# nv-tlabs/GEN3C

Measured on NVIDIA H100. Metric: denoise-steps/sec, 7B DiT, 121-frame 720p latent, higher is better.
Workload: dtype bf16

## Files before the change

### gen3c_b200/_lib.py

```python
from __future__ import annotations

import ctypes as C
import os
from pathlib import Path

_HERE = Path(__file__).resolve().parent
LIB_PATH = _HERE / "lib" / "libgen3c_b200.so"


class G3CError(RuntimeError):
    pass


class DitConfig(C.Structure):
    _fields_ = [
        ("model_channels", C.c_int),
        ("num_blocks", C.c_int),
        ("num_heads", C.c_int),
        ("ffn_dim", C.c_int),
        ("context_dim", C.c_int),
        ("adaln_lora_dim", C.c_int),
        ("in_channels", C.c_int),
        ("out_channels", C.c_int),
        ("concat_padding_mask", C.c_int),
# ... 23 lines not shown
        ("sigma_data", C.c_float),
        ("sigma_aug", C.c_float),
        ("guidance", C.c_float),
        ("xt_next", C.c_void_p),
        ("cond_mask_uncond", C.c_void_p),
        ("net_output", C.c_void_p),
    ]


_P = C.c_void_p
_I = C.c_int
_F = C.c_float

SIGNATURES = {
    "g3c_last_error": (C.c_char_p, []),
    "g3c_version": (_I, []),
    "g3c_device_info": (_I, [C.POINTER(_I), C.POINTER(_I), C.POINTER(_I)]),
    "g3c_render_create": (_I, [_I, _I, _I, C.POINTER(_P)]),
    "g3c_render_destroy": (_I, [_P]),
    "g3c_render_set_deterministic": (_I, [_P, _I]),
    "g3c_forward_warp": (_I, [_P, _P, _P, _P, _P, _P, _I, _I, _I, _P, _P, _P, _P, _P]),
    "g3c_render_cache": (_I, [_P, _P, _P, _P, _P, _P, _I, _I, _I, _I, _I, _P, _P, _P, _P]),
    "g3c_bilinear_splatting": (_I, [_P, _P, _P, _P, _P, _I, _I, _I, _P, _P, _P]),
    "g3c_splat_indices": (_I, [_P, _I, _I, _I, _P, _P]),
    "g3c_unproject_points": (_I, [_P, _P, _P, _P, _I, _I, _I, _I, _P, _P]),
    "g3c_reliable_depth_mask": (_I, [_P, _I, _I, _I, _I, _F, _F, _P, _P]),
    "g3c_align_depth_nonrigid": (_I, [_P, _P, _P, _P, _P, _I, _I, _I, _F, _F, _P, _P]),
    "g3c_foreground_occlusion": (_I, [_P, _P, _P, _P, _I, _I, _I, _I, _P, _P, _P, _P]),
    "g3c_render_cache_occlusion": (_I, [_P, _P, _P, _P, _I, _I, _I, _I, _P, _P, _P, _I, _I, _P]),
    "g3c_gemm_bf16": (_I, [_P, _P, _P, _I, _I, _I, _I, _I, _I, _I, _P, _I, _P]),
    "g3c_gemm_norm_rope_bf16": (_I, [_P, _P, _P, _I, _I, _I, _I, _I, _I, _P, _P, _F, _P]),
    "g3c_quantize_rows_fp8": (_I, [_P, _I, _I, _I, _P, _I, _P, _P]),
    "g3c_gemm_fp8": (_I, [_P, _P, _P, _P, _P, _I, _I, _I, _I, _I, _I, _I, _P, _I, _P]),
    "g3c_gemm_norm_rope_fp8": (_I, [_P, _P, _P, _P, _P, _I, _I, _I, _I, _I, _I, _P, _P, _F, _P]),
    "g3c_ln_modulate_fp8": (_I, [_P, _P, _P, _P, _P, _P, _I, _I, _F, _P]),
    "g3c_attn_fwd": (_I, [_P, _P, _P, _P, _I, _I, _I, _I, _I, _I, _I, _F, _P]),
    "g3c_attn_fwd_sbhd": (_I, [_P, _P, _P, _P, _I, _I, _I, _I, _I, _I, _I, _I, _F, _P]),
    "g3c_attn_set_trace": (_I, [_P]),
    "g3c_ln_modulate": (_I, [_P, _P, _P, _P, _P, _I, _I, _F, _P]),
    "g3c_rmsnorm_rope": (_I, [_P, _I, _I, _I, _P, _P, _F, _P]),
    "g3c_dit_create": (_I, [C.POINTER(DitConfig), C.POINTER(_P)]),
    "g3c_dit_destroy": (_I, [_P]),
    "g3c_dit_load": (_I, [_P, C.c_char_p, _P, C.POINTER(C.c_int64), _I, _I]),
    "g3c_nccl_unique_id": (_I, [_P]),
    "g3c_dit_enable_cp": (_I, [_P, _P, _I, _I]),
    "g3c_dit_cp_export": (_I, [_P, _P]),
    "g3c_dit_cp_import": (_I, [_P, _P, _I]),
    "g3c_dit_cp_mode": (_I, [_P]),
    "g3c_dit_disable_cp": (_I, [_P]),
    "g3c_dit_set_linear_fp8": (_I, [_P, _I]),
    "g3c_dit_enable_cfg_parallel": (_I, [_P, _I]),
    "g3c_dit_cfg_export": (_I, [_P, _P]),
    "g3c_dit_cfg_import": (_I, [_P, _P]),
    "g3c_dit_set_shape": (_I, [_P, _I, _I, _I, _I, _F]),
    "g3c_dit_forward": (_I, [_P, _P, _P, _P, _P, _F, _P, _P, _P]),
    "g3c_denoise_step": (_I, [_P, C.POINTER(StepArgs), _P]),
    "g3c_dit_profile": (_I, [_P, _I]),
    "g3c_dit_profile_read": (_I, [_P, C.POINTER(_F), C.POINTER(_I), _I]),
    "g3c_dit_profile_wait_ms": (_I, [_P, C.POINTER(_F)]),
    "g3c_dit_workspace_bytes": (C.c_int64, [_P]),
    "g3c_dit_last_launch_count": (_I, [_P]),
    "g3c_dit_read_tables": (_I, [_P, _I, _P, _P, _P]),
    "g3c_dit_read_modulation": (_I, [_P, _F, _P, _P, _P]),
    "g3c_dit_read_step": (_I, [_P, _P, _P, _P, _P, _P]),
    "g3c_attn_fwd_gated": (_I, [_P, _P, _P, _P, _I, _I, _I, _I, _I, _I, _I, _F, _P, C.c_uint32, _I, _P, _P]),
}

# ... 41 lines not shown
```

### gen3c_b200/csrc/common.cuh

```cuda
#pragma once
#include <cuda.h>
#include <cuda_bf16.h>
#include <cuda_runtime.h>
#include <stdint.h>
#include <stdio.h>

#include "../../include/gen3c_b200.h"
#include "wgmma_ops.cuh"

namespace g3c {

void set_error(const char* fmt, ...);
int cuda_fail(cudaError_t e, const char* what, const char* file, int line);
#define G3C_CUDA(x)                                                         \
  do {                                                                      \
    cudaError_t _e = (x);                                                   \
    if (_e != cudaSuccess) return ::g3c::cuda_fail(_e, #x, __FILE__, __LINE__); \
  } while (0)
#define G3C_REQUIRE(cond, ...)        \
  do {                                \
    if (!(cond)) {                    \
      ::g3c::set_error(__VA_ARGS__);  \
      return G3C_EINVAL;       \
    }                                 \
// ... 11 lines not shown
__device__ __forceinline__ uint32_t smem_u32(const void* p) {
  return static_cast<uint32_t>(__cvta_generic_to_shared(p));
}
__device__ __forceinline__ uint32_t lane_id() { return threadIdx.x & 31; }
__device__ __forceinline__ uint32_t warp_id() { return __shfl_sync(0xffffffffu, threadIdx.x >> 5, 0); }

__device__ __forceinline__ bool elect_one() {
  uint32_t pred = 0;
  asm volatile(
      "{\n\t.reg .pred P;\n\t"
      "elect.sync _|P, 0xffffffff;\n\t"
      "selp.b32 %0, 1, 0, P;\n\t}\n"
      : "=r"(pred));
  return pred != 0;
}

__device__ __forceinline__ void mbar_init(uint64_t* bar, uint32_t count) {
  asm volatile("mbarrier.init.shared::cta.b64 [%0], %1;\n" ::"r"(smem_u32(bar)), "r"(count));
}
__device__ __forceinline__ void fence_barrier_init() {
  asm volatile("fence.mbarrier_init.release.cluster;\n" ::: "memory");
}
__device__ __forceinline__ void fence_proxy_async() {
  asm volatile("fence.proxy.async.shared::cta;\n" ::: "memory");
}
__device__ __forceinline__ void mbar_expect_tx(uint64_t* bar, uint32_t bytes) {
  asm volatile("mbarrier.arrive.expect_tx.shared::cta.b64 _, [%0], %1;\n" ::"r"(smem_u32(bar)),
               "r"(bytes)
               : "memory");
}
__device__ __forceinline__ void mbar_arrive(uint64_t* bar) {
  asm volatile("mbarrier.arrive.shared::cta.b64 _, [%0];\n" ::"r"(smem_u32(bar)) : "memory");
}
#ifndef G3C_MBAR_SUSPEND_NS
#define G3C_MBAR_SUSPEND_NS 0
#endif
__device__ __forceinline__ bool mbar_try_wait(uint64_t* bar, uint32_t parity) {
  uint32_t ok;
#if G3C_MBAR_SUSPEND_NS > 0
  asm volatile(
      "{\n\t.reg .pred P;\n\t"
      "mbarrier.try_wait.parity.shared::cta.b64 P, [%1], %2, %3;\n\t"
      "selp.b32 %0, 1, 0, P;\n\t}\n"
      : "=r"(ok)
      : "r"(smem_u32(bar)), "r"(parity), "r"((uint32_t)G3C_MBAR_SUSPEND_NS)
      : "memory");
#else
  asm volatile(
      "{\n\t.reg .pred P;\n\t"
      "mbarrier.try_wait.parity.shared::cta.b64 P, [%1], %2;\n\t"
      "selp.b32 %0, 1, 0, P;\n\t}\n"
      : "=r"(ok)
      : "r"(smem_u32(bar)), "r"(parity)
      : "memory");
#endif
  return ok != 0;
}
__device__ __forceinline__ bool mbar_test(uint64_t* bar, uint32_t parity) {
  uint32_t ok;
  asm volatile(
      "{\n\t.reg .pred P;\n\t"
      "mbarrier.test_wait.parity.shared::cta.b64 P, [%1], %2;\n\t"
      "selp.b32 %0, 1, 0, P;\n\t}\n"
      : "=r"(ok)
      : "r"(smem_u32(bar)), "r"(parity)
      : "memory");
  return ok != 0;
}
#ifndef G3C_MBAR_TIMEOUT_NS
#define G3C_MBAR_TIMEOUT_NS 4000000000ull
#endif
__device__ __forceinline__ uint64_t global_timer_ns() {
  uint64_t t;
  asm volatile("mov.u64 %0, %%globaltimer;\n" : "=l"(t));
  return t;
}
#ifdef G3C_MBAR_DEBUG
#define G3C_MBAR_TIMEOUT_ACTION(bar, parity)                                                                 \
  do {                                                                                                       \
    printf("g3c: mbarrier timeout block(%d,%d) thread %d bar@%u parity %u\n", blockIdx.x, blockIdx.y,        \
           threadIdx.x, bar, parity);                                                                        \
    __trap();                                                                                                \
  } while (0)
#else
#define G3C_MBAR_TIMEOUT_ACTION(bar, parity) asm volatile("trap;\n")
#endif
__device__ __forceinline__ void mbar_wait(uint64_t* bar, uint32_t parity) {
  if (mbar_try_wait(bar, parity)) return;
  uint32_t spins = 0;
  uint64_t t0 = 0;
  while (!mbar_try_wait(bar, parity)) {
    if ((++spins & 0xFFFu) == 0) {
      uint64_t now = global_timer_ns();
      if (t0 == 0) t0 = now;
      else if (now - t0 > G3C_MBAR_TIMEOUT_NS) G3C_MBAR_TIMEOUT_ACTION(smem_u32(bar), parity);
    }
  }
}

__device__ __forceinline__ void mbar_wait_ns(uint64_t* bar, uint32_t parity, unsigned long long timeout_ns) {
  if (mbar_try_wait(bar, parity)) return;
  uint32_t spins = 0;
  uint64_t t0 = 0;
  while (!mbar_try_wait(bar, parity)) {
    if ((++spins & 0xFFFu) == 0) {
      uint64_t now = global_timer_ns();
      if (t0 == 0) t0 = now;
      else if (now - t0 > timeout_ns) G3C_MBAR_TIMEOUT_ACTION(smem_u32(bar), parity);
    }
  }
}

__device__ __forceinline__ void mbar_wait_ns_or_exit(uint64_t* bar, uint32_t parity, unsigned long long timeout_ns) {
  if (mbar_try_wait(bar, parity)) return;
  uint32_t spins = 0;
  uint64_t t0 = 0;
  while (!mbar_try_wait(bar, parity)) {
    if ((++spins & 0xFFFu) == 0) {
      uint64_t now = global_timer_ns();
      if (t0 == 0) t0 = now;
      else if (now - t0 > timeout_ns) asm volatile("exit;\n");
    }
  }
}

__device__ __forceinline__ void tma_prefetch_desc(const CUtensorMap* m) {
  asm volatile("prefetch.tensormap [%0];\n" ::"l"(reinterpret_cast<uint64_t>(m)) : "memory");
}
__device__ __forceinline__ void tma_load_2d(void* smem_dst, const CUtensorMap* m, uint64_t* bar,
                                            int c0, int c1) {
  asm volatile(
      "cp.async.bulk.tensor.2d.shared::cluster.global.mbarrier::complete_tx::bytes"
      " [%0], [%1, {%3, %4}], [%2];\n" ::"r"(smem_u32(smem_dst)),
      "l"(reinterpret_cast<uint64_t>(m)), "r"(smem_u32(bar)), "r"(c0), "r"(c1)
      : "memory");
}
__device__ __forceinline__ void tma_load_3d(void* smem_dst, const CUtensorMap* m, uint64_t* bar,
                                            int c0, int c1, int c2) {
  asm volatile(
      "cp.async.bulk.tensor.3d.shared::cluster.global.mbarrier::complete_tx::bytes"
      " [%0], [%1, {%3, %4, %5}], [%2];\n" ::"r"(smem_u32(smem_dst)),
      "l"(reinterpret_cast<uint64_t>(m)), "r"(smem_u32(bar)), "r"(c0), "r"(c1), "r"(c2)
      : "memory");
}

__device__ __forceinline__ void tma_store_2d(const CUtensorMap* m, const void* smem_src, int c0, int c1) {
  asm volatile("cp.async.bulk.tensor.2d.global.shared::cta.bulk_group [%0, {%2, %3}], [%1];\n" ::"l"(
                   reinterpret_cast<uint64_t>(m)),
               "r"(smem_u32(smem_src)), "r"(c0), "r"(c1)
               : "memory");
}
__device__ __forceinline__ void tma_reduce_add_2d(const CUtensorMap* m, const void* smem_src, int c0, int c1) {
  asm volatile("cp.reduce.async.bulk.tensor.2d.global.shared::cta.add.bulk_group [%0, {%2, %3}], [%1];\n" ::"l"(
                   reinterpret_cast<uint64_t>(m)),
               "r"(smem_u32(smem_src)), "r"(c0), "r"(c1)
               : "memory");
}
__device__ __forceinline__ void tma_store_commit() { asm volatile("cp.async.bulk.commit_group;\n" ::: "memory"); }
template <int N>
__device__ __forceinline__ void tma_store_wait_read() {
  asm volatile("cp.async.bulk.wait_group.read %0;\n" ::"n"(N) : "memory");
}
template <int N>
__device__ __forceinline__ void tma_store_wait_all() {
  asm volatile("cp.async.bulk.wait_group %0;\n" ::"n"(N) : "memory");
}

__device__ __forceinline__ void wgmma_fence() { asm volatile("wgmma.fence.sync.aligned;\n" ::: "memory"); }
__device__ __forceinline__ void wgmma_commit() { asm volatile("wgmma.commit_group.sync.aligned;\n" ::: "memory"); }
// ... 62 lines not shown
```

### gen3c_b200/csrc/gemm_wgmma.cu

```cuda
#include <cstdlib>
#include <cstring>

#include "kernels.h"

namespace g3c {

constexpr int BM = 128;
constexpr int BK = 64;
constexpr int WG_K = 16;
template <bool kFp8>
constexpr int kBlockK = kFp8 ? 2 * BK : BK;
constexpr int GEMM_THREADS = 384;

struct GemmParams {
  int M, N, K;
  int ldd;
  void* D;
  const float* gate;
  int num_m_blk, num_n_blk, num_k_blk;
  int super_n;
  const float* nr_gamma;
  const float* nr_cs;
  float nr_eps;
  const float* scale_a;
  const float* scale_b;
};

constexpr int EPI_NORM_ROPE_BF16 = 4;

template <int BN>
struct GemmSmem {
  static constexpr int kABytes = BM * BK * 2;
  static constexpr int kBBytes = BN * BK * 2;
  static constexpr int kStageBytes = kABytes + kBBytes;
  static constexpr int kStages = (192 * 1024) / kStageBytes;
  static constexpr int kBarBytes = 256;
  static constexpr int kTotal = kStages * kStageBytes + kBarBytes + 1024;
};

__device__ __forceinline__ float gelu_erf(float x) {
  return 0.5f * x * (1.0f + erff(x * 0.70710678118654752440f));
}

__device__ __forceinline__ void tile_coords(const GemmParams& p, int tile, int& m_blk, int& n_blk) {
  int per_super = p.num_m_blk * p.super_n;
  int sc = tile / per_super;
  int rem = tile - sc * per_super;
  int n0 = sc * p.super_n;
  int width = p.num_n_blk - n0 < p.super_n ? p.num_n_blk - n0 : p.super_n;
  m_blk = rem / width;
  n_blk = n0 + rem - m_blk * width;
}

template <int BN>
__device__ __forceinline__ void epilogue_norm_rope(const float (&acc)[BN / 2], const GemmParams& p, int row_a, int col_q,
                                                   int n_base) {
#pragma unroll
  for (int hd = 0; hd < BN / 128; ++hd) {
    if (n_base + hd * 128 >= p.N) break;
    float ss[2] = {0.f, 0.f};
#pragma unroll
    for (int i = 16 * hd; i < 16 * hd + 16; ++i) {
      ss[0] = fmaf(acc[4 * i], acc[4 * i], fmaf(acc[4 * i + 1], acc[4 * i + 1], ss[0]));
      ss[1] = fmaf(acc[4 * i + 2], acc[4 * i + 2], fmaf(acc[4 * i + 3], acc[4 * i + 3], ss[1]));
    }
#pragma unroll
    for (int h = 0; h < 2; ++h) {
      ss[h] += __shfl_xor_sync(0xffffffffu, ss[h], 1);
      ss[h] += __shfl_xor_sync(0xffffffffu, ss[h], 2);
    }
#pragma unroll
    for (int h = 0; h < 2; ++h) {
      const int row = row_a + 8 * h;
      if (row >= p.M) continue;
      const float rstd = rsqrtf(ss[h] * (1.0f / 128.0f) + p.nr_eps);
      const float* cs = p.nr_cs ? p.nr_cs + (size_t)row * 128 : nullptr;
      __nv_bfloat16* dptr = reinterpret_cast<__nv_bfloat16*>(p.D) + (size_t)row * p.ldd + n_base + hd * 128;
#pragma unroll
      for (int i = 0; i < 8; ++i) {
        const int c = 8 * i + col_q;
        const float2 ga = *reinterpret_cast<const float2*>(p.nr_gamma + c);
        const float2 gb = *reinterpret_cast<const float2*>(p.nr_gamma + 64 + c);
        const int ia = 4 * (16 * hd + i) + 2 * h, ib = 4 * (16 * hd + i + 8) + 2 * h;
        float a[2] = {acc[ia] * (rstd * ga.x), acc[ia + 1] * (rstd * ga.y)};
// ... 51 lines not shown
        if (col >= p.N) continue;
        const bool pair = col + 1 < p.N;
        float v0 = acc[4 * i + 2 * h], v1 = acc[4 * i + 2 * h + 1];
        if constexpr (EPI == G3C_EPI_BF16 || EPI == G3C_EPI_GELU_BF16) {
          if constexpr (EPI == G3C_EPI_GELU_BF16) {
            v0 = gelu_erf(v0);
            v1 = gelu_erf(v1);
          }
          __nv_bfloat16* dptr = reinterpret_cast<__nv_bfloat16*>(p.D) + (size_t)row * p.ldd + col;
          if (pair) *reinterpret_cast<uint32_t*>(dptr) = pack_bf16x2(v0, v1);
          else dptr[0] = __float2bfloat16_rn(v0);
        } else {
          float* dptr = reinterpret_cast<float*>(p.D) + (size_t)row * p.ldd + col;
          if constexpr (EPI == G3C_EPI_GATED_RESIDUAL_F32) {
            if (pair) {
              const float2 g = *reinterpret_cast<const float2*>(p.gate + col);
              float2 x = *reinterpret_cast<float2*>(dptr);
              x.x = fmaf(g.x, v0, x.x);
              x.y = fmaf(g.y, v1, x.y);
              *reinterpret_cast<float2*>(dptr) = x;
            } else {
              dptr[0] = fmaf(p.gate[col], v0, dptr[0]);
            }
          } else {
            if (pair) *reinterpret_cast<float2*>(dptr) = make_float2(v0, v1);
            else dptr[0] = v0;
          }
        }
      }
    }
  }
}

template <int BN, int EPI, bool kFp8>
__global__ void __launch_bounds__(GEMM_THREADS, 1)
    k_gemm(const __grid_constant__ CUtensorMap tmA, const __grid_constant__ CUtensorMap tmB, const GemmParams p) {
  using S = GemmSmem<BN>;
  constexpr int kStages = S::kStages;
  extern __shared__ uint8_t smem_raw[];
  uint8_t* smem = reinterpret_cast<uint8_t*>((reinterpret_cast<uintptr_t>(smem_raw) + 1023) &
                                             ~static_cast<uintptr_t>(1023));
  uint8_t* smem_a = smem;
  uint8_t* smem_b = smem + kStages * S::kABytes;
  uint64_t* bars = reinterpret_cast<uint64_t*>(smem + kStages * S::kStageBytes);
  uint64_t* full = bars;
  uint64_t* empty = bars + kStages;

  const uint32_t wg = threadIdx.x / 128;
  const uint32_t tid = threadIdx.x % 128;

  if (threadIdx.x == 0) {
    tma_prefetch_desc(&tmA);
    tma_prefetch_desc(&tmB);
    for (int i = 0; i < kStages; ++i) {
      mbar_init(&full[i], 1);
      mbar_init(&empty[i], 2);
    }
    fence_barrier_init();
  }
  __syncthreads();

  const int num_tiles = p.num_m_blk * p.num_n_blk;

  if (wg == 0) {
    setmaxnreg_dec<40>();
    if (tid == 0) {
      uint32_t stage = 0, phase = 0;
      for (int tile = blockIdx.x; tile < num_tiles; tile += gridDim.x) {
        int m_blk, n_blk;
        tile_coords(p, tile, m_blk, n_blk);
        for (int kb = 0; kb < p.num_k_blk; ++kb) {
          mbar_wait(&empty[stage], phase ^ 1);
          mbar_expect_tx(&full[stage], S::kStageBytes);
          tma_load_2d(smem_a + stage * S::kABytes, &tmA, &full[stage], kb * kBlockK<kFp8>, m_blk * BM);
          tma_load_2d(smem_b + stage * S::kBBytes, &tmB, &full[stage], kb * kBlockK<kFp8>, n_blk * BN);
          if (++stage == kStages) {
            stage = 0;
            phase ^= 1;
          }
        }
      }
    }
  } else {
    setmaxnreg_inc<232>();
    const uint32_t c = wg - 1;
    const uint32_t warp = tid / 32, lane = tid % 32;
    uint32_t stage = 0, phase = 0;
    float acc[BN / 2];
    for (int tile = blockIdx.x; tile < num_tiles; tile += gridDim.x) {
      int m_blk, n_blk;
      tile_coords(p, tile, m_blk, n_blk);
      if constexpr (kFp8) {
        static_assert(BN <= 128, "fp8 tiles hold two accumulator sets");
        float part[BN / 2];
#pragma unroll
        for (int i = 0; i < BN / 2; ++i) acc[i] = 0.f;
        for (int kb = 0; kb < p.num_k_blk; ++kb) {
          mbar_wait(&full[stage], phase);
          const uint64_t da = make_sdesc_sw128(smem_u32(smem_a + stage * S::kABytes + c * 64 * 128));
          const uint64_t db = make_sdesc_sw128(smem_u32(smem_b + stage * S::kBBytes));
          wgmma_fence();
#pragma unroll
          for (int k = 0; k < BK / WG_K; ++k) {
            const uint64_t a = sdesc_advance(da, k * WG_K * 2), b = sdesc_advance(db, k * WG_K * 2);
            if constexpr (BN == 128) wgmma_ss_n128_e4m3(part, a, b, k != 0 ? 1u : 0u);
            else wgmma_ss_n64_e4m3(part, a, b, k != 0 ? 1u : 0u);
          }
          wgmma_commit();
          wgmma_wait<0>();
          fence_regs(part);
          if (tid == 0) mbar_arrive(&empty[stage]);
#pragma unroll
          for (int i = 0; i < BN / 2; ++i) acc[i] += part[i];
          if (++stage == kStages) {
            stage = 0;
            phase ^= 1;
          }
        }
      } else {
        uint32_t prev_stage = 0;
        for (int kb = 0; kb < p.num_k_blk; ++kb) {
          mbar_wait(&full[stage], phase);
          const uint64_t da = make_sdesc_sw128(smem_u32(smem_a + stage * S::kABytes + c * 64 * 128));
          const uint64_t db = make_sdesc_sw128(smem_u32(smem_b + stage * S::kBBytes));
          wgmma_fence();
#pragma unroll
          for (int k = 0; k < BK / WG_K; ++k) {
            const uint64_t a = sdesc_advance(da, k * WG_K * 2), b = sdesc_advance(db, k * WG_K * 2);
            const uint32_t accumulate = (kb | k) != 0 ? 1u : 0u;
            if constexpr (BN == 256) wgmma_ss_n256(acc, a, b, accumulate);
            else if constexpr (BN == 128) wgmma_ss_n128(acc, a, b, accumulate);
            else wgmma_ss_n64(acc, a, b, accumulate);
          }
          wgmma_commit();
          wgmma_wait<1>();
          fence_regs(acc);
          if (kb > 0 && tid == 0) mbar_arrive(&empty[prev_stage]);
          prev_stage = stage;
          if (++stage == kStages) {
            stage = 0;
            phase ^= 1;
          }
        }
        wgmma_wait<0>();
        fence_regs(acc);
        if (tid == 0) mbar_arrive(&empty[prev_stage]);
      }
      const int row_a = m_blk * BM + (int)(c * 64 + warp * 16 + lane / 4), col_q = (int)(2 * (lane % 4));
      if constexpr (kFp8) dequantise<BN>(acc, p, row_a, col_q, n_blk * BN);
      epilogue<BN, EPI>(acc, p, row_a, col_q, n_blk * BN);
    }
  }
}

template <int BN, int EPI, bool kFp8>
static int launch_gemm(const CUtensorMap& tmA, const CUtensorMap& tmB, const GemmParams& p, cudaStream_t st) {
  using S = GemmSmem<BN>;
  static bool configured = false;
  if (!configured) {
    G3C_CUDA(cudaFuncSetAttribute(k_gemm<BN, EPI, kFp8>, cudaFuncAttributeMaxDynamicSharedMemorySize, S::kTotal));
    configured = true;
  }
  int tiles = p.num_m_blk * p.num_n_blk;
  int grid = tiles < sm_count() ? tiles : sm_count();
  k_gemm<BN, EPI, kFp8><<<grid, GEMM_THREADS, S::kTotal, st>>>(tmA, tmB, p);
  G3C_CUDA(cudaGetLastError());
  return G3C_OK;
}

template <int BN, bool kFp8>
static int dispatch_epi(int epi, const CUtensorMap& tmA, const CUtensorMap& tmB, const GemmParams& p, cudaStream_t st) {
  switch (epi) {
    case G3C_EPI_BF16: return launch_gemm<BN, G3C_EPI_BF16, kFp8>(tmA, tmB, p, st);
    case G3C_EPI_GELU_BF16: return launch_gemm<BN, G3C_EPI_GELU_BF16, kFp8>(tmA, tmB, p, st);
    case G3C_EPI_GATED_RESIDUAL_F32: return launch_gemm<BN, G3C_EPI_GATED_RESIDUAL_F32, kFp8>(tmA, tmB, p, st);
    case G3C_EPI_F32: return launch_gemm<BN, G3C_EPI_F32, kFp8>(tmA, tmB, p, st);
    case EPI_NORM_ROPE_BF16:
      if constexpr (BN >= 128) return launch_gemm<BN, EPI_NORM_ROPE_BF16, kFp8>(tmA, tmB, p, st);
      break;
  }
  set_error("gemm: unknown epilogue %d", epi);
  return G3C_EINVAL;
}

static int gemm_any(const void* A, const void* B, const float* scale_a, const float* scale_b, void* D, int M, int N,
                    int K, int lda, int ldb, int ldd, int epilogue, const float* gate, int block_n, cudaStream_t st,
                    const NormRope* norm_rope) {
  const bool fp8 = scale_a != nullptr;
  G3C_REQUIRE(A && B && D, "gemm: null operand");
  G3C_REQUIRE(epilogue >= G3C_EPI_BF16 && epilogue <= G3C_EPI_F32, "gemm: unknown epilogue %d", epilogue);
  if (norm_rope) {
    G3C_REQUIRE(epilogue == G3C_EPI_BF16 && N % 128 == 0 && norm_rope->gamma,
                "gemm: the RMSNorm/RoPE epilogue needs the bf16 epilogue, N %% 128 == 0 and a gain vector");
    G3C_REQUIRE((reinterpret_cast<uintptr_t>(norm_rope->gamma) & 15) == 0 &&
                    (reinterpret_cast<uintptr_t>(norm_rope->cs) & 15) == 0,
                "gemm: RMSNorm gain / RoPE table must be 16-byte aligned");
    epilogue = EPI_NORM_ROPE_BF16;
  }
  G3C_REQUIRE(M > 0 && N > 0 && K > 0, "gemm: bad shape %dx%dx%d", M, N, K);
  if (fp8)
    G3C_REQUIRE(K % 16 == 0 && lda % 16 == 0 && ldb % 16 == 0, "gemm_fp8: K/lda/ldb must be multiples of 16");
  else
    G3C_REQUIRE(K % 8 == 0 && lda % 8 == 0 && ldb % 8 == 0, "gemm: K/lda/ldb must be multiples of 8");
  G3C_REQUIRE(lda >= K && ldb >= K && ldd >= N, "gemm: leading dimension smaller than extent");
  if (epilogue == G3C_EPI_BF16 || epilogue == G3C_EPI_GELU_BF16 || epilogue == EPI_NORM_ROPE_BF16)
    G3C_REQUIRE(ldd % 8 == 0 && (reinterpret_cast<uintptr_t>(D) & 15) == 0,
                "gemm: bf16 output needs ldd %% 8 == 0 and 16-byte aligned base");
  else
    G3C_REQUIRE(ldd % 4 == 0 && (reinterpret_cast<uintptr_t>(D) & 15) == 0,
                "gemm: f32 output needs ldd %% 4 == 0 and 16-byte aligned base");
  G3C_REQUIRE(epilogue != G3C_EPI_GATED_RESIDUAL_F32 ||
                  (gate && (reinterpret_cast<uintptr_t>(gate) & 15) == 0),
              "gemm: gated-residual epilogue needs a 16-byte aligned gate vector");
  int bn = block_n;
  G3C_REQUIRE(bn == 0 || bn == 64 || bn == 128 || bn == 256 || bn == 512, "gemm: block_n %d unsupported", bn);
  if (bn == 512) {
    G3C_REQUIRE(N % 256 == 0, "gemm: block_n 512 needs N %% 256 == 0 (N=%d)", N);
    bn = 256;
  }
  if (bn == 0) bn = (N >= 256 && N % 256 == 0) ? 256 : (N > 64 ? 128 : 64);
  if (fp8 && bn == 256) bn = 128;
  G3C_REQUIRE(epilogue != EPI_NORM_ROPE_BF16 || bn >= 128, "gemm: the RMSNorm/RoPE epilogue needs tiles of whole heads");

  CUtensorMap tmA, tmB;
  const int esize = fp8 ? 1 : 2, bk = fp8 ? kBlockK<true> : kBlockK<false>;
  const CUtensorMapDataType dt = fp8 ? CU_TENSOR_MAP_DATA_TYPE_UINT8 : CU_TENSOR_MAP_DATA_TYPE_BFLOAT16;
  uint64_t dimsA[2] = {(uint64_t)K, (uint64_t)M}, strA[1] = {(uint64_t)lda * esize};
  uint32_t boxA[2] = {(uint32_t)bk, BM};
  int rc = make_tmap_bf16_sw128(&tmA, A, 2, dimsA, strA, boxA, dt);
  if (rc) return rc;
  uint64_t dimsB[2] = {(uint64_t)K, (uint64_t)N}, strB[1] = {(uint64_t)ldb * esize};
  uint32_t boxB[2] = {(uint32_t)bk, (uint32_t)bn};
  rc = make_tmap_bf16_sw128(&tmB, B, 2, dimsB, strB, boxB, dt);
  if (rc) return rc;

  GemmParams p;
  p.M = M;
  p.N = N;
  p.K = K;
  p.ldd = ldd;
  p.D = D;
  p.gate = gate;
  p.nr_gamma = norm_rope ? norm_rope->gamma : nullptr;
  p.nr_cs = norm_rope ? norm_rope->cs : nullptr;
  p.nr_eps = norm_rope ? norm_rope->eps : 0.0f;
  p.scale_a = scale_a;
  p.scale_b = scale_b;
  p.num_m_blk = (M + BM - 1) / BM;
  p.num_n_blk = (N + bn - 1) / bn;
  p.num_k_blk = (K + bk - 1) / bk;
  long long col_bytes = (long long)bn * K * esize;
  int sn = (int)((16ll << 20) / (col_bytes > 0 ? col_bytes : 1));
  if (sn < 1) sn = 1;
  if (sn > p.num_n_blk) sn = p.num_n_blk;
  p.super_n = sn;
  if (fp8) return bn == 64 ? dispatch_epi<64, true>(epilogue, tmA, tmB, p, st)
                           : dispatch_epi<128, true>(epilogue, tmA, tmB, p, st);
  switch (bn) {
    case 64: return dispatch_epi<64, false>(epilogue, tmA, tmB, p, st);
    case 128: return dispatch_epi<128, false>(epilogue, tmA, tmB, p, st);
    default: return dispatch_epi<256, false>(epilogue, tmA, tmB, p, st);
  }
}

int gemm_bf16(const void* A, const void* B, void* D, int M, int N, int K, int lda, int ldb, int ldd,
              int epilogue, const float* gate, int block_n, cudaStream_t st, const NormRope* norm_rope) {
  return gemm_any(A, B, nullptr, nullptr, D, M, N, K, lda, ldb, ldd, epilogue, gate, block_n, st, norm_rope);
}

int gemm_fp8(const void* A8, const float* scale_a, const void* B8, const float* scale_b, void* D, int M, int N, int K,
             int lda, int ldb, int ldd, int epilogue, const float* gate, int block_n, cudaStream_t st,
             const NormRope* norm_rope) {
  G3C_REQUIRE(scale_a && scale_b, "gemm_fp8: null scale vector");
  G3C_REQUIRE((reinterpret_cast<uintptr_t>(scale_a) & 15) == 0 && (reinterpret_cast<uintptr_t>(scale_b) & 15) == 0,
              "gemm_fp8: scale vectors must be 16-byte aligned");
  return gemm_any(A8, B8, scale_a, scale_b, D, M, N, K, lda, ldb, ldd, epilogue, gate, block_n, st, norm_rope);
}

}

extern "C" int g3c_gemm_bf16(const void* A, const void* B, void* D, int M, int N, int K, int lda,
                             int ldb, int ldd, int epilogue, const float* gate, int block_n,
                             void* stream) {
  return g3c::gemm_bf16(A, B, D, M, N, K, lda, ldb, ldd, epilogue, gate, block_n,
                        (cudaStream_t)stream);
}

extern "C" int g3c_gemm_fp8(const void* A8, const float* scale_A, const void* B8, const float* scale_B, void* D, int M,
                            int N, int K, int lda, int ldb, int ldd, int epilogue, const float* gate, int block_n,
                            void* stream) {
  return g3c::gemm_fp8(A8, scale_A, B8, scale_B, D, M, N, K, lda, ldb, ldd, epilogue, gate, block_n,
                       (cudaStream_t)stream);
}

extern "C" int g3c_gemm_norm_rope_fp8(const void* A8, const float* scale_A, const void* B8, const float* scale_B, void* D,
                                      int M, int N, int K, int lda, int ldb, int ldd, const float* gamma,
                                      const float* cos_sin, float eps, void* stream) {
  g3c::NormRope nr;
  nr.gamma = gamma;
  nr.cs = cos_sin;
  nr.eps = eps;
  return g3c::gemm_fp8(A8, scale_A, B8, scale_B, D, M, N, K, lda, ldb, ldd, G3C_EPI_BF16, nullptr, 0,
                       (cudaStream_t)stream, &nr);
}

extern "C" int g3c_gemm_norm_rope_bf16(const void* A, const void* B, void* D, int M, int N, int K, int lda, int ldb,
                                       int ldd, const float* gamma, const float* cos_sin, float eps, void* stream) {
  g3c::NormRope nr;
  nr.gamma = gamma;
  nr.cs = cos_sin;
  nr.eps = eps;
  return g3c::gemm_bf16(A, B, D, M, N, K, lda, ldb, ldd, G3C_EPI_BF16, nullptr, 0, (cudaStream_t)stream, &nr);
}
```

### include/gen3c_b200.h

```cpp
#ifndef GEN3C_B200_H_
#define GEN3C_B200_H_

#include <stdint.h>

#ifdef __cplusplus
extern "C" {
#endif

#define G3C_OK 0
#define G3C_EINVAL (-1)
#define G3C_ECUDA (-2)
#define G3C_ENOMEM (-3)
#define G3C_ESTATE (-4)
#define G3C_ENCCL (-5)

const char* g3c_last_error(void);
int g3c_version(void);
int g3c_device_info(int* sm_count, int* cc_major, int* cc_minor);


typedef struct g3c_render g3c_render_t;

int g3c_render_create(int H, int W, int max_items_per_pass, g3c_render_t** out);
int g3c_render_destroy(g3c_render_t* r);
// ... 21 lines not shown
int g3c_unproject_points(const float* depth, const float* w2c, const float* K, const uint8_t* mask,
                         int b, int H, int W, int is_depth, float* points, void* stream);

int g3c_reliable_depth_mask(const float* depth, int b, int H, int W, int window, float ratio_thresh,
                            float eps, uint8_t* out, void* stream);

int g3c_align_depth_nonrigid(const float* depth, const float* target_depth, const uint8_t* target_mask, const float* K,
                             const float* c2w, int H, int W, int num_iters, float lambda_arap, float lr,
                             float* out_depth, void* stream);

int g3c_foreground_occlusion(const float* points, const unsigned char* boundary, const float* w2c, const float* K, int b,
                             int C, int H, int W, float* warped, float* mask, float* depth, void* stream);

int g3c_render_cache_occlusion(const float* points, const unsigned char* boundary, const float* w2cs, const float* Ks, int B,
                               int F_target, int N, int src_frames, float* pixels, float* masks, float* depth, int H, int W,
                               void* stream);


#define G3C_EPI_BF16 0
#define G3C_EPI_GELU_BF16 1
#define G3C_EPI_GATED_RESIDUAL_F32 2
#define G3C_EPI_F32 3

int g3c_gemm_bf16(const void* A, const void* B, void* D, int M, int N, int K, int lda, int ldb,
                  int ldd, int epilogue, const float* gate, int block_n, void* stream);

int g3c_gemm_norm_rope_bf16(const void* A, const void* B, void* D, int M, int N, int K, int lda, int ldb, int ldd,
                            const float* gamma, const float* cos_sin, float eps, void* stream);

int g3c_quantize_rows_fp8(const void* x_bf16, int ld, int R, int C, void* codes, int ldq, float* scales, void* stream);

int g3c_gemm_fp8(const void* A8, const float* scale_A, const void* B8, const float* scale_B, void* D, int M, int N,
                 int K, int lda, int ldb, int ldd, int epilogue, const float* gate, int block_n, void* stream);

int g3c_gemm_norm_rope_fp8(const void* A8, const float* scale_A, const void* B8, const float* scale_B, void* D, int M,
                           int N, int K, int lda, int ldb, int ldd, const float* gamma, const float* cos_sin, float eps,
                           void* stream);

int g3c_attn_fwd(const void* q, const void* k, const void* vt, void* o, int Lq, int Lk, int heads,
                 int ldq, int ldk, int ldo, int vt_chunk_len, float scale, void* stream);

int g3c_attn_fwd_sbhd(const void* q, const void* k, const void* v, void* o, int Lq, int Lk, int batch, int heads,
                      int ldq, int ldk, int ldv, int ldo, float scale, void* stream);

int g3c_attn_set_trace(unsigned long long* device_buffer);

int g3c_ln_modulate(float* x, const void* pos_bf16, const float* shift, const float* scale,
                    void* y_bf16, int L, int D, float eps, void* stream);

int g3c_ln_modulate_fp8(float* x, const void* pos_bf16, const float* shift, const float* scale, void* y_codes,
                        float* y_scales, int L, int D, float eps, void* stream);

int g3c_rmsnorm_rope(void* qk_bf16, int ld, int L, int heads, const float* gamma,
                     const float* cos_sin, float eps, void* stream);

typedef struct g3c_dit g3c_dit_t;

typedef struct g3c_dit_config {
  int model_channels;
  int num_blocks;
  int num_heads;
  int ffn_dim;
  int context_dim;
  int adaln_lora_dim;
  int in_channels;
  int out_channels;
// ... 72 lines not shown
```

Baseline: 0.1371.

## Launch GEMM as 2-CTA clusters with TMA multicast of shared B tiles

The persistent wgmma GEMM now runs as 2-CTA thread-block clusters. Each cluster processes two adjacent M blocks against the same N block. Each CTA TMA-loads half of the B tile and multicasts it to both CTAs' shared memory, and the empty-stage barriers are released across the cluster. This roughly halves global/L2 traffic for the weight operand. In exchange it adds cross-CTA barrier coupling, cluster-scheduling limits on the grid size (computed via occupancy query), and a possible wasted half-cluster when the M block count is odd. A small query entry point reporting the last launch's grid and cluster size is also added.

New measurement: 0.1379 (median of 6 runs). No clear change (+0.6%).

```diff
diff --git a/gen3c_b200/_lib.py b/gen3c_b200/_lib.py
--- a/gen3c_b200/_lib.py
+++ b/gen3c_b200/_lib.py
@@ -80,6 +80,7 @@
     "g3c_quantize_rows_fp8": (_I, [_P, _I, _I, _I, _P, _I, _P, _P]),
     "g3c_gemm_fp8": (_I, [_P, _P, _P, _P, _P, _I, _I, _I, _I, _I, _I, _I, _P, _I, _P]),
     "g3c_gemm_norm_rope_fp8": (_I, [_P, _P, _P, _P, _P, _I, _I, _I, _I, _I, _I, _P, _P, _F, _P]),
+    "g3c_gemm_last_launch": (_I, [C.POINTER(_I), C.POINTER(_I), C.POINTER(_I)]),
     "g3c_ln_modulate_fp8": (_I, [_P, _P, _P, _P, _P, _P, _I, _I, _F, _P]),
     "g3c_attn_fwd": (_I, [_P, _P, _P, _P, _I, _I, _I, _I, _I, _I, _I, _F, _P]),
     "g3c_attn_fwd_sbhd": (_I, [_P, _P, _P, _P, _I, _I, _I, _I, _I, _I, _I, _I, _F, _P]),
diff --git a/gen3c_b200/csrc/common.cuh b/gen3c_b200/csrc/common.cuh
--- a/gen3c_b200/csrc/common.cuh
+++ b/gen3c_b200/csrc/common.cuh
@@ -133,6 +133,23 @@
   }
 }
 
+__device__ __forceinline__ uint32_t cluster_ctarank() {
+  uint32_t r;
+  asm volatile("mov.u32 %0, %%cluster_ctarank;\n" : "=r"(r));
+  return r;
+}
+__device__ __forceinline__ void cluster_sync() {
+  asm volatile("barrier.cluster.arrive.release;\nbarrier.cluster.wait.acquire;\n" ::: "memory");
+}
+__device__ __forceinline__ uint32_t mapa_shared(uint32_t p, uint32_t cta) {
+  uint32_t r;
+  asm volatile("mapa.shared::cluster.u32 %0, %1, %2;\n" : "=r"(r) : "r"(p), "r"(cta));
+  return r;
+}
+__device__ __forceinline__ void mbar_arrive_cluster(uint32_t cluster_addr) {
+  asm volatile("mbarrier.arrive.shared::cluster.b64 _, [%0];\n" ::"r"(cluster_addr) : "memory");
+}
+
 __device__ __forceinline__ void mbar_wait_ns(uint64_t* bar, uint32_t parity, unsigned long long timeout_ns) {
   if (mbar_try_wait(bar, parity)) return;
   uint32_t spins = 0;
@@ -170,6 +187,14 @@
       "l"(reinterpret_cast<uint64_t>(m)), "r"(smem_u32(bar)), "r"(c0), "r"(c1)
       : "memory");
 }
+__device__ __forceinline__ void tma_load_2d_multicast(void* smem_dst, const CUtensorMap* m, uint64_t* bar, int c0,
+                                                      int c1, uint16_t cta_mask) {
+  asm volatile(
+      "cp.async.bulk.tensor.2d.shared::cluster.global.mbarrier::complete_tx::bytes.multicast::cluster"
+      " [%0], [%1, {%4, %5}], [%2], %3;\n" ::"r"(smem_u32(smem_dst)),
+      "l"(reinterpret_cast<uint64_t>(m)), "r"(smem_u32(bar)), "h"(cta_mask), "r"(c0), "r"(c1)
+      : "memory");
+}
 __device__ __forceinline__ void tma_load_3d(void* smem_dst, const CUtensorMap* m, uint64_t* bar,
                                             int c0, int c1, int c2) {
   asm volatile(
diff --git a/gen3c_b200/csrc/gemm_wgmma.cu b/gen3c_b200/csrc/gemm_wgmma.cu
--- a/gen3c_b200/csrc/gemm_wgmma.cu
+++ b/gen3c_b200/csrc/gemm_wgmma.cu
@@ -11,6 +11,7 @@
 template <bool kFp8>
 constexpr int kBlockK = kFp8 ? 2 * BK : BK;
 constexpr int GEMM_THREADS = 384;
+constexpr int kCluster = 2;
 
 struct GemmParams {
   int M, N, K;
@@ -42,14 +43,18 @@
   return 0.5f * x * (1.0f + erff(x * 0.70710678118654752440f));
 }
 
-__device__ __forceinline__ void tile_coords(const GemmParams& p, int tile, int& m_blk, int& n_blk) {
-  int per_super = p.num_m_blk * p.super_n;
-  int sc = tile / per_super;
-  int rem = tile - sc * per_super;
+__host__ __device__ __forceinline__ int num_pairs(const GemmParams& p) {
+  return (p.num_m_blk + kCluster - 1) / kCluster * p.num_n_blk;
+}
+__device__ __forceinline__ void pair_coords(const GemmParams& p, int pair, uint32_t rank, int& m_blk, int& n_blk) {
+  int per_super = (p.num_m_blk + kCluster - 1) / kCluster * p.super_n;
+  int sc = pair / per_super;
+  int rem = pair - sc * per_super;
   int n0 = sc * p.super_n;
   int width = p.num_n_blk - n0 < p.super_n ? p.num_n_blk - n0 : p.super_n;
-  m_blk = rem / width;
-  n_blk = n0 + rem - m_blk * width;
+  const int m_pair = rem / width;
+  n_blk = n0 + rem - m_pair * width;
+  m_blk = kCluster * m_pair + (int)rank;
 }
 
 template <int BN>
@@ -183,32 +188,35 @@
 
   const uint32_t wg = threadIdx.x / 128;
   const uint32_t tid = threadIdx.x % 128;
+  const uint32_t rank = cluster_ctarank();
+  const int cluster = blockIdx.x / kCluster, num_clusters = gridDim.x / kCluster;
 
   if (threadIdx.x == 0) {
     tma_prefetch_desc(&tmA);
     tma_prefetch_desc(&tmB);
     for (int i = 0; i < kStages; ++i) {
       mbar_init(&full[i], 1);
-      mbar_init(&empty[i], 2);
+      mbar_init(&empty[i], 2 * kCluster);
     }
     fence_barrier_init();
   }
-  __syncthreads();
-
-  const int num_tiles = p.num_m_blk * p.num_n_blk;
+  cluster_sync();
+
+  const int pairs = num_pairs(p);
 
   if (wg == 0) {
     setmaxnreg_dec<40>();
     if (tid == 0) {
       uint32_t stage = 0, phase = 0;
-      for (int tile = blockIdx.x; tile < num_tiles; tile += gridDim.x) {
+      for (int pair = cluster; pair < pairs; pair += num_clusters) {
         int m_blk, n_blk;
-        tile_coords(p, tile, m_blk, n_blk);
+        pair_coords(p, pair, rank, m_blk, n_blk);
         for (int kb = 0; kb < p.num_k_blk; ++kb) {
           mbar_wait(&empty[stage], phase ^ 1);
           mbar_expect_tx(&full[stage], S::kStageBytes);
           tma_load_2d(smem_a + stage * S::kABytes, &tmA, &full[stage], kb * kBlockK<kFp8>, m_blk * BM);
-          tma_load_2d(smem_b + stage * S::kBBytes, &tmB, &full[stage], kb * kBlockK<kFp8>, n_blk * BN);
+          tma_load_2d_multicast(smem_b + stage * S::kBBytes + rank * (S::kBBytes / 2), &tmB, &full[stage],
+                                kb * kBlockK<kFp8>, n_blk * BN + (int)rank * (BN / 2), 0x3);
           if (++stage == kStages) {
             stage = 0;
             phase ^= 1;
@@ -220,11 +228,18 @@
     setmaxnreg_inc<232>();
     const uint32_t c = wg - 1;
     const uint32_t warp = tid / 32, lane = tid % 32;
+    const uint32_t empty0 = mapa_shared(smem_u32(empty), 0), empty1 = mapa_shared(smem_u32(empty), 1);
+    auto release = [&](uint32_t s) {
+      if (tid == 0) {
+        mbar_arrive_cluster(empty0 + 8 * s);
+        mbar_arrive_cluster(empty1 + 8 * s);
+      }
+    };
     uint32_t stage = 0, phase = 0;
     float acc[BN / 2];
-    for (int tile = blockIdx.x; tile < num_tiles; tile += gridDim.x) {
+    for (int pair = cluster; pair < pairs; pair += num_clusters) {
       int m_blk, n_blk;
-      tile_coords(p, tile, m_blk, n_blk);
+      pair_coords(p, pair, rank, m_blk, n_blk);
       if constexpr (kFp8) {
         static_assert(BN <= 128, "fp8 tiles hold two accumulator sets");
         float part[BN / 2];
@@ -244,7 +259,7 @@
           wgmma_commit();
           wgmma_wait<0>();
           fence_regs(part);
-          if (tid == 0) mbar_arrive(&empty[stage]);
+          release(stage);
 #pragma unroll
           for (int i = 0; i < BN / 2; ++i) acc[i] += part[i];
           if (++stage == kStages) {
@@ -270,7 +285,7 @@
           wgmma_commit();
           wgmma_wait<1>();
           fence_regs(acc);
-          if (kb > 0 && tid == 0) mbar_arrive(&empty[prev_stage]);
+          if (kb > 0) release(prev_stage);
           prev_stage = stage;
           if (++stage == kStages) {
             stage = 0;
@@ -279,27 +294,46 @@
         }
         wgmma_wait<0>();
         fence_regs(acc);
-        if (tid == 0) mbar_arrive(&empty[prev_stage]);
+        release(prev_stage);
       }
       const int row_a = m_blk * BM + (int)(c * 64 + warp * 16 + lane / 4), col_q = (int)(2 * (lane % 4));
       if constexpr (kFp8) dequantise<BN>(acc, p, row_a, col_q, n_blk * BN);
       epilogue<BN, EPI>(acc, p, row_a, col_q, n_blk * BN);
     }
   }
-}
+  cluster_sync();
+}
+
+struct GemmLaunch {
+  int grid, cluster_size, max_clusters;
+};
+static thread_local GemmLaunch g_last_launch = {0, 0, 0};
 
 template <int BN, int EPI, bool kFp8>
 static int launch_gemm(const CUtensorMap& tmA, const CUtensorMap& tmB, const GemmParams& p, cudaStream_t st) {
   using S = GemmSmem<BN>;
-  static bool configured = false;
-  if (!configured) {
+  cudaLaunchAttribute attr;
+  attr.id = cudaLaunchAttributeClusterDimension;
+  attr.val.clusterDim.x = kCluster;
+  attr.val.clusterDim.y = 1;
+  attr.val.clusterDim.z = 1;
+  cudaLaunchConfig_t cfg = {};
+  cfg.gridDim = dim3(kCluster);
+  cfg.blockDim = dim3(GEMM_THREADS);
+  cfg.dynamicSmemBytes = S::kTotal;
+  cfg.stream = st;
+  cfg.attrs = &attr;
+  cfg.numAttrs = 1;
+  static int max_clusters = 0;
+  if (max_clusters == 0) {
     G3C_CUDA(cudaFuncSetAttribute(k_gemm<BN, EPI, kFp8>, cudaFuncAttributeMaxDynamicSharedMemorySize, S::kTotal));
-    configured = true;
-  }
-  int tiles = p.num_m_blk * p.num_n_blk;
-  int grid = tiles < sm_count() ? tiles : sm_count();
-  k_gemm<BN, EPI, kFp8><<<grid, GEMM_THREADS, S::kTotal, st>>>(tmA, tmB, p);
-  G3C_CUDA(cudaGetLastError());
+    G3C_CUDA(cudaOccupancyMaxActiveClusters(&max_clusters, k_gemm<BN, EPI, kFp8>, &cfg));
+    G3C_REQUIRE(max_clusters > 0, "gemm: no cluster of %d CTAs fits on the device", kCluster);
+  }
+  const int pairs = num_pairs(p);
+  cfg.gridDim = dim3(kCluster * (pairs < max_clusters ? pairs : max_clusters));
+  G3C_CUDA(cudaLaunchKernelEx(&cfg, k_gemm<BN, EPI, kFp8>, tmA, tmB, p));
+  g_last_launch = {(int)cfg.gridDim.x, kCluster, max_clusters};
   return G3C_OK;
 }
 
@@ -365,7 +399,7 @@
   int rc = make_tmap_bf16_sw128(&tmA, A, 2, dimsA, strA, boxA, dt);
   if (rc) return rc;
   uint64_t dimsB[2] = {(uint64_t)K, (uint64_t)N}, strB[1] = {(uint64_t)ldb * esize};
-  uint32_t boxB[2] = {(uint32_t)bk, (uint32_t)bn};
+  uint32_t boxB[2] = {(uint32_t)bk, (uint32_t)(bn / kCluster)};
   rc = make_tmap_bf16_sw128(&tmB, B, 2, dimsB, strB, boxB, dt);
   if (rc) return rc;
 
@@ -414,6 +448,13 @@
 
 }
 
+extern "C" int g3c_gemm_last_launch(int* grid, int* cluster_size, int* max_clusters) {
+  if (grid) *grid = g3c::g_last_launch.grid;
+  if (cluster_size) *cluster_size = g3c::g_last_launch.cluster_size;
+  if (max_clusters) *max_clusters = g3c::g_last_launch.max_clusters;
+  return G3C_OK;
+}
+
 extern "C" int g3c_gemm_bf16(const void* A, const void* B, void* D, int M, int N, int K, int lda,
                              int ldb, int ldd, int epilogue, const float* gate, int block_n,
                              void* stream) {
diff --git a/include/gen3c_b200.h b/include/gen3c_b200.h
--- a/include/gen3c_b200.h
+++ b/include/gen3c_b200.h
@@ -77,6 +77,8 @@
 
 int g3c_gemm_fp8(const void* A8, const float* scale_A, const void* B8, const float* scale_B, void* D, int M, int N,
                  int K, int lda, int ldb, int ldd, int epilogue, const float* gate, int block_n, void* stream);
+
+int g3c_gemm_last_launch(int* grid, int* cluster_size, int* max_clusters);
 
 int g3c_gemm_norm_rope_fp8(const void* A8, const float* scale_A, const void* B8, const float* scale_B, void* D, int M,
                            int N, int K, int lda, int ldb, int ldd, const float* gamma, const float* cos_sin, float eps,
```

## Launch GEMM as 2-CTA clusters sharing the B tile via TMA multicast

Applied to the files above, without the earlier changes.

The persistent wgmma GEMM now runs as 2-CTA clusters. Each CTA in a pair computes an adjacent M block, and the two CTAs split the B (weight) tile load, multicasting each half to both CTAs. The intent is to halve L2/HBM traffic for the weight operand and raise effective load bandwidth. In exchange, stage release now needs cross-CTA mbarrier arrivals and cluster syncs, which couple the pair's pipelines. Scheduling is limited to whole clusters and may leave some SMs idle, and when the M block count is odd the extra CTA may read out of range.

Result: no change. 0.1354 before, 0.1361 after (median of 6 runs) (+0.5%).

```diff
diff --git a/gen3c_b200/_lib.py b/gen3c_b200/_lib.py
--- a/gen3c_b200/_lib.py
+++ b/gen3c_b200/_lib.py
@@ -79,6 +79,7 @@
     "g3c_gemm_norm_rope_bf16": (_I, [_P, _P, _P, _I, _I, _I, _I, _I, _I, _P, _P, _F, _P]),
     "g3c_quantize_rows_fp8": (_I, [_P, _I, _I, _I, _P, _I, _P, _P]),
     "g3c_gemm_fp8": (_I, [_P, _P, _P, _P, _P, _I, _I, _I, _I, _I, _I, _I, _P, _I, _P]),
+    "g3c_gemm_max_clusters": (_I, [_I, _I, C.POINTER(_I)]),
     "g3c_gemm_norm_rope_fp8": (_I, [_P, _P, _P, _P, _P, _I, _I, _I, _I, _I, _I, _P, _P, _F, _P]),
     "g3c_ln_modulate_fp8": (_I, [_P, _P, _P, _P, _P, _P, _I, _I, _F, _P]),
     "g3c_attn_fwd": (_I, [_P, _P, _P, _P, _I, _I, _I, _I, _I, _I, _I, _F, _P]),
diff --git a/gen3c_b200/csrc/common.cuh b/gen3c_b200/csrc/common.cuh
--- a/gen3c_b200/csrc/common.cuh
+++ b/gen3c_b200/csrc/common.cuh
@@ -67,6 +67,31 @@
 __device__ __forceinline__ void mbar_arrive(uint64_t* bar) {
   asm volatile("mbarrier.arrive.shared::cta.b64 _, [%0];\n" ::"r"(smem_u32(bar)) : "memory");
 }
+
+__device__ __forceinline__ uint32_t cluster_ctarank() {
+  uint32_t r;
+  asm volatile("mov.u32 %0, %%cluster_ctarank;\n" : "=r"(r));
+  return r;
+}
+__device__ __forceinline__ uint32_t cluster_id_x() {
+  uint32_t r;
+  asm volatile("mov.u32 %0, %%clusterid.x;\n" : "=r"(r));
+  return r;
+}
+__device__ __forceinline__ uint32_t cluster_count_x() {
+  uint32_t r;
+  asm volatile("mov.u32 %0, %%nclusterid.x;\n" : "=r"(r));
+  return r;
+}
+__device__ __forceinline__ void cluster_sync() {
+  asm volatile("barrier.cluster.arrive.release;\n" ::: "memory");
+  asm volatile("barrier.cluster.wait.acquire;\n" ::: "memory");
+}
+__device__ __forceinline__ void mbar_arrive_cluster(uint64_t* bar, uint32_t cta) {
+  uint32_t remote;
+  asm volatile("mapa.shared::cluster.u32 %0, %1, %2;\n" : "=r"(remote) : "r"(smem_u32(bar)), "r"(cta));
+  asm volatile("mbarrier.arrive.shared::cluster.b64 _, [%0];\n" ::"r"(remote) : "memory");
+}
 #ifndef G3C_MBAR_SUSPEND_NS
 #define G3C_MBAR_SUSPEND_NS 0
 #endif
@@ -170,6 +195,14 @@
       "l"(reinterpret_cast<uint64_t>(m)), "r"(smem_u32(bar)), "r"(c0), "r"(c1)
       : "memory");
 }
+__device__ __forceinline__ void tma_load_2d_multicast(void* smem_dst, const CUtensorMap* m, uint64_t* bar, int c0,
+                                                      int c1, uint16_t cta_mask) {
+  asm volatile(
+      "cp.async.bulk.tensor.2d.shared::cluster.global.mbarrier::complete_tx::bytes.multicast::cluster"
+      " [%0], [%1, {%3, %4}], [%2], %5;\n" ::"r"(smem_u32(smem_dst)),
+      "l"(reinterpret_cast<uint64_t>(m)), "r"(smem_u32(bar)), "r"(c0), "r"(c1), "h"(cta_mask)
+      : "memory");
+}
 __device__ __forceinline__ void tma_load_3d(void* smem_dst, const CUtensorMap* m, uint64_t* bar,
                                             int c0, int c1, int c2) {
   asm volatile(
diff --git a/gen3c_b200/csrc/gemm_wgmma.cu b/gen3c_b200/csrc/gemm_wgmma.cu
--- a/gen3c_b200/csrc/gemm_wgmma.cu
+++ b/gen3c_b200/csrc/gemm_wgmma.cu
@@ -42,14 +42,16 @@
   return 0.5f * x * (1.0f + erff(x * 0.70710678118654752440f));
 }
 
-__device__ __forceinline__ void tile_coords(const GemmParams& p, int tile, int& m_blk, int& n_blk) {
-  int per_super = p.num_m_blk * p.super_n;
+__device__ __forceinline__ int num_pair_rows(const GemmParams& p) { return (p.num_m_blk + 1) / 2; }
+
+__device__ __forceinline__ void tile_coords(const GemmParams& p, int tile, int& pm, int& n_blk) {
+  int per_super = num_pair_rows(p) * p.super_n;
   int sc = tile / per_super;
   int rem = tile - sc * per_super;
   int n0 = sc * p.super_n;
   int width = p.num_n_blk - n0 < p.super_n ? p.num_n_blk - n0 : p.super_n;
-  m_blk = rem / width;
-  n_blk = n0 + rem - m_blk * width;
+  pm = rem / width;
+  n_blk = n0 + rem - pm * width;
 }
 
 template <int BN>
@@ -167,6 +169,11 @@
   }
 }
 
+__device__ __forceinline__ void release_stage(uint64_t* empty, uint32_t peer) {
+  mbar_arrive(empty);
+  mbar_arrive_cluster(empty, peer);
+}
+
 template <int BN, int EPI, bool kFp8>
 __global__ void __launch_bounds__(GEMM_THREADS, 1)
     k_gemm(const __grid_constant__ CUtensorMap tmA, const __grid_constant__ CUtensorMap tmB, const GemmParams p) {
@@ -183,32 +190,36 @@
 
   const uint32_t wg = threadIdx.x / 128;
   const uint32_t tid = threadIdx.x % 128;
+  const uint32_t rank = cluster_ctarank(), peer = rank ^ 1u;
 
   if (threadIdx.x == 0) {
     tma_prefetch_desc(&tmA);
     tma_prefetch_desc(&tmB);
     for (int i = 0; i < kStages; ++i) {
       mbar_init(&full[i], 1);
-      mbar_init(&empty[i], 2);
+      mbar_init(&empty[i], 4);
     }
     fence_barrier_init();
   }
-  __syncthreads();
-
-  const int num_tiles = p.num_m_blk * p.num_n_blk;
+  cluster_sync();
+
+  const int num_tiles = num_pair_rows(p) * p.num_n_blk;
+  const int first_tile = (int)cluster_id_x(), tile_step = (int)cluster_count_x();
 
   if (wg == 0) {
     setmaxnreg_dec<40>();
     if (tid == 0) {
       uint32_t stage = 0, phase = 0;
-      for (int tile = blockIdx.x; tile < num_tiles; tile += gridDim.x) {
-        int m_blk, n_blk;
-        tile_coords(p, tile, m_blk, n_blk);
+      for (int tile = first_tile; tile < num_tiles; tile += tile_step) {
+        int pm, n_blk;
+        tile_coords(p, tile, pm, n_blk);
+        const int m_blk = 2 * pm + (int)rank;
         for (int kb = 0; kb < p.num_k_blk; ++kb) {
           mbar_wait(&empty[stage], phase ^ 1);
           mbar_expect_tx(&full[stage], S::kStageBytes);
           tma_load_2d(smem_a + stage * S::kABytes, &tmA, &full[stage], kb * kBlockK<kFp8>, m_blk * BM);
-          tma_load_2d(smem_b + stage * S::kBBytes, &tmB, &full[stage], kb * kBlockK<kFp8>, n_blk * BN);
+          tma_load_2d_multicast(smem_b + stage * S::kBBytes + rank * (BN / 2) * 128, &tmB, &full[stage],
+                                kb * kBlockK<kFp8>, n_blk * BN + (int)rank * (BN / 2), 0b11);
           if (++stage == kStages) {
             stage = 0;
             phase ^= 1;
@@ -216,15 +227,17 @@
         }
       }
     }
+    __syncwarp();
   } else {
     setmaxnreg_inc<232>();
     const uint32_t c = wg - 1;
     const uint32_t warp = tid / 32, lane = tid % 32;
     uint32_t stage = 0, phase = 0;
     float acc[BN / 2];
-    for (int tile = blockIdx.x; tile < num_tiles; tile += gridDim.x) {
-      int m_blk, n_blk;
-      tile_coords(p, tile, m_blk, n_blk);
+    for (int tile = first_tile; tile < num_tiles; tile += tile_step) {
+      int pm, n_blk;
+      tile_coords(p, tile, pm, n_blk);
+      const int m_blk = 2 * pm + (int)rank;
       if constexpr (kFp8) {
         static_assert(BN <= 128, "fp8 tiles hold two accumulator sets");
         float part[BN / 2];
@@ -244,7 +257,7 @@
           wgmma_commit();
           wgmma_wait<0>();
           fence_regs(part);
-          if (tid == 0) mbar_arrive(&empty[stage]);
+          if (tid == 0) release_stage(&empty[stage], peer);
 #pragma unroll
           for (int i = 0; i < BN / 2; ++i) acc[i] += part[i];
           if (++stage == kStages) {
@@ -270,7 +283,7 @@
           wgmma_commit();
           wgmma_wait<1>();
           fence_regs(acc);
-          if (kb > 0 && tid == 0) mbar_arrive(&empty[prev_stage]);
+          if (kb > 0 && tid == 0) release_stage(&empty[prev_stage], peer);
           prev_stage = stage;
           if (++stage == kStages) {
             stage = 0;
@@ -279,27 +292,58 @@
         }
         wgmma_wait<0>();
         fence_regs(acc);
-        if (tid == 0) mbar_arrive(&empty[prev_stage]);
+        if (tid == 0) release_stage(&empty[prev_stage], peer);
       }
       const int row_a = m_blk * BM + (int)(c * 64 + warp * 16 + lane / 4), col_q = (int)(2 * (lane % 4));
       if constexpr (kFp8) dequantise<BN>(acc, p, row_a, col_q, n_blk * BN);
       epilogue<BN, EPI>(acc, p, row_a, col_q, n_blk * BN);
     }
   }
+  cluster_sync();
+}
+
+static cudaLaunchConfig_t cluster_launch_config(cudaLaunchAttribute* attr, int smem_bytes, cudaStream_t st) {
+  attr[0].id = cudaLaunchAttributeClusterDimension;
+  attr[0].val.clusterDim.x = 2;
+  attr[0].val.clusterDim.y = 1;
+  attr[0].val.clusterDim.z = 1;
+  cudaLaunchConfig_t cfg = {};
+  cfg.blockDim = dim3(GEMM_THREADS);
+  cfg.dynamicSmemBytes = smem_bytes;
+  cfg.stream = st;
+  cfg.attrs = attr;
+  cfg.numAttrs = 1;
+  return cfg;
+}
+
+template <int BN, int EPI, bool kFp8>
+static int max_clusters(int* out) {
+  static int clusters = 0;
+  if (clusters == 0) {
+    G3C_CUDA(cudaFuncSetAttribute(k_gemm<BN, EPI, kFp8>, cudaFuncAttributeMaxDynamicSharedMemorySize,
+                                  GemmSmem<BN>::kTotal));
+    cudaLaunchAttribute attr[1];
+    cudaLaunchConfig_t cfg = cluster_launch_config(attr, GemmSmem<BN>::kTotal, 0);
+    cfg.gridDim = dim3(2 * sm_count());
+    int n = 0;
+    G3C_CUDA(cudaOccupancyMaxActiveClusters(&n, k_gemm<BN, EPI, kFp8>, &cfg));
+    G3C_REQUIRE(n > 0, "gemm: no 2-CTA cluster of this kernel fits on the device");
+    clusters = n;
+  }
+  *out = clusters;
+  return G3C_OK;
 }
 
 template <int BN, int EPI, bool kFp8>
 static int launch_gemm(const CUtensorMap& tmA, const CUtensorMap& tmB, const GemmParams& p, cudaStream_t st) {
-  using S = GemmSmem<BN>;
-  static bool configured = false;
-  if (!configured) {
-    G3C_CUDA(cudaFuncSetAttribute(k_gemm<BN, EPI, kFp8>, cudaFuncAttributeMaxDynamicSharedMemorySize, S::kTotal));
-    configured = true;
-  }
-  int tiles = p.num_m_blk * p.num_n_blk;
-  int grid = tiles < sm_count() ? tiles : sm_count();
-  k_gemm<BN, EPI, kFp8><<<grid, GEMM_THREADS, S::kTotal, st>>>(tmA, tmB, p);
-  G3C_CUDA(cudaGetLastError());
+  int clusters = 0;
+  int rc = max_clusters<BN, EPI, kFp8>(&clusters);
+  if (rc) return rc;
+  const int pair_tiles = (p.num_m_blk + 1) / 2 * p.num_n_blk;
+  cudaLaunchAttribute attr[1];
+  cudaLaunchConfig_t cfg = cluster_launch_config(attr, GemmSmem<BN>::kTotal, st);
+  cfg.gridDim = dim3(2 * (pair_tiles < clusters ? pair_tiles : clusters));
+  G3C_CUDA(cudaLaunchKernelEx(&cfg, k_gemm<BN, EPI, kFp8>, tmA, tmB, p));
   return G3C_OK;
 }
 
@@ -365,7 +409,7 @@
   int rc = make_tmap_bf16_sw128(&tmA, A, 2, dimsA, strA, boxA, dt);
   if (rc) return rc;
   uint64_t dimsB[2] = {(uint64_t)K, (uint64_t)N}, strB[1] = {(uint64_t)ldb * esize};
-  uint32_t boxB[2] = {(uint32_t)bk, (uint32_t)bn};
+  uint32_t boxB[2] = {(uint32_t)bk, (uint32_t)bn / 2};
   rc = make_tmap_bf16_sw128(&tmB, B, 2, dimsB, strB, boxB, dt);
   if (rc) return rc;
 
@@ -421,6 +465,20 @@
                         (cudaStream_t)stream);
 }
 
+extern "C" int g3c_gemm_max_clusters(int block_n, int fp8, int* clusters) {
+  G3C_REQUIRE(clusters, "gemm_max_clusters: null output");
+  if (fp8) {
+    if (block_n == 64) return g3c::max_clusters<64, G3C_EPI_BF16, true>(clusters);
+    if (block_n == 128) return g3c::max_clusters<128, G3C_EPI_BF16, true>(clusters);
+  } else {
+    if (block_n == 64) return g3c::max_clusters<64, G3C_EPI_BF16, false>(clusters);
+    if (block_n == 128) return g3c::max_clusters<128, G3C_EPI_BF16, false>(clusters);
+    if (block_n == 256) return g3c::max_clusters<256, G3C_EPI_BF16, false>(clusters);
+  }
+  g3c::set_error("gemm_max_clusters: no %s tile of %d columns", fp8 ? "fp8" : "bf16", block_n);
+  return G3C_EINVAL;
+}
+
 extern "C" int g3c_gemm_fp8(const void* A8, const float* scale_A, const void* B8, const float* scale_B, void* D, int M,
                             int N, int K, int lda, int ldb, int ldd, int epilogue, const float* gate, int block_n,
                             void* stream) {
diff --git a/include/gen3c_b200.h b/include/gen3c_b200.h
--- a/include/gen3c_b200.h
+++ b/include/gen3c_b200.h
@@ -77,6 +77,8 @@
 
 int g3c_gemm_fp8(const void* A8, const float* scale_A, const void* B8, const float* scale_B, void* D, int M, int N,
                  int K, int lda, int ldb, int ldd, int epilogue, const float* gate, int block_n, void* stream);
+
+int g3c_gemm_max_clusters(int block_n, int fp8, int* clusters);
 
 int g3c_gemm_norm_rope_fp8(const void* A8, const float* scale_A, const void* B8, const float* scale_B, void* D, int M,
                            int N, int K, int lda, int ldb, int ldd, const float* gamma, const float* cos_sin, float eps,
```
